# jcasal-homer/HomerHEVC

Hardware: AMD Instinct MI355X
Metric: encoded frames/sec, 1080p & 2160p YUV420 fixed-QP IPPP, 1/2/4/8 MI355X (higher is better)
Workload: dtype int16; 1 GPU; cfg2-1080p-encode; sequences_per_gpu=256, width=1920, height=1080, wfpp_num_threads=17, qp=32, gop=IPPP intra_period=100

## Files before the change

### homerhevc_amd/csrc/enc/enc_common.h

```cpp
#pragma once
#include "enc_prims.h"
#if !defined(__HIPCC__)
#include <stdio.h>
#include <stdlib.h>
#endif

#if !defined(__HIPCC__) && defined(HENC_TRACE_ENABLE)
#include <stdio.h>
extern "C" FILE *henc_trace_file;
#define HENC_TRACE(...) do { if (henc_trace_file) fprintf(henc_trace_file, __VA_ARGS__); } while (0)
#define HENC_TRACE_PW(e, tag)                                                                                                                      \
	do {                                                                                                                                       \
		if (henc_trace_file) {                                                                                                             \
			unsigned a_[3] = {0, 0, 0};                                                                                                \
			for (int c_ = 0; c_ < 3; c_++) {                                                                                           \
				const int n_ = c_ ? 32 : 64;                                                                                       \
				const pred_t *p_ = c_ ? (e).w->pred_c[c_ - 1] : (e).w->pred_y;                                                     \
				for (int y_ = 0; y_ < n_; y_++)                                                                                    \
					for (int x_ = 0; x_ < n_; x_++) a_[c_] += (unsigned)(p_[y_ * n_ + x_] & 0xffff) * (unsigned)(1 + ((x_ + 3 * y_) & 7)); \
			}                                                                                                                          \
			fprintf(henc_trace_file, "PW %s ctu=%d pred=%u,%u,%u\n", tag, (e).ctu->ctu_number, a_[0], a_[1], a_[2]);                   \
		}                                                                                                                                  \
	} while (0)
#else
// ... 200 lines not shown
	e.bg_node = -1;
	*mode = uni(b->bg_mode);
	*bits = uni(b->bg_bits);
	return true;
#else
	(void)g; (void)e; (void)ni; (void)mode; (void)bits;
	return false;
#endif
}

#if defined(__HIP_DEVICE_COMPILE__)
#define HENC_HELPERS(e) true
#else
#define HENC_HELPERS(e) false
#endif

template <class G>
HENC_INLINE bool rd_full(const G, const Seq &S) { return G::rdfull && S.rd_mode == RDM_FULL; }

struct DepthState {
	uint32_t bits = 0;
	HENC_INLINE int get(int d) const { return (int)((bits >> (4 * d)) & 15u); }
	HENC_INLINE void set(int d, int v) { bits = (bits & ~(15u << (4 * d))) | ((uint32_t)v << (4 * d)); }
	HENC_INLINE void inc(int d) { bits += 1u << (4 * d); }
};
struct DepthCosts {
	uint32_t v0 = 0, v1 = 0, v2 = 0, v3 = 0, v4 = 0;
	HENC_INLINE uint32_t get(int d) const { return d == 0 ? v0 : (d == 1 ? v1 : (d == 2 ? v2 : (d == 3 ? v3 : v4))); }
	HENC_INLINE void set(int d, uint32_t x) { v0 = d == 0 ? x : v0; v1 = d == 1 ? x : v1; v2 = d == 2 ? x : v2; v3 = d == 3 ? x : v3; v4 = d == 4 ? x : v4; }
	HENC_INLINE void add(int d, uint32_t x) { set(d, get(d) + x); }
};

struct DepthInts4 {
	int v0 = 0, v1 = 0, v2 = 0, v3 = 0;
	HENC_INLINE int get(int i) const { return i == 0 ? v0 : (i == 1 ? v1 : (i == 2 ? v2 : v3)); }
	HENC_INLINE void set(int i, int x) { v0 = i == 0 ? x : v0; v1 = i == 1 ? x : v1; v2 = i == 2 ? x : v2; v3 = i == 3 ? x : v3; }
	HENC_INLINE void add(int i, int x) { set(i, get(i) + x); }
};

HENC_INLINE int raster2abs(int r)
{
	const int x = r & 15, y = r >> 4;
	int a = 0;
	for (int b = 0; b < 4; b++) a |= (((x >> b) & 1) << (2 * b)) | (((y >> b) & 1) << (2 * b + 1));
	return a;
}
HENC_INLINE int abs2raster(int a)
{
	int x = 0, y = 0;
	for (int b = 0; b < 4; b++) {
		x |= ((a >> (2 * b)) & 1) << b;
		y |= ((a >> (2 * b + 1)) & 1) << b;
	}
	return y * 16 + x;
}
HENC_INLINE Node &node_of(Enc &__restrict__ e, int idx)
{
	HENC_ENC_IN_LDS(e);
#if !defined(__HIPCC__)
	if (idx >= NODES_RESIDENT && node_quadrant(idx) != e.node_quad) {
		fprintf(stderr, "node_of: node %d of quadrant %d while quadrant %d is resident\n", idx, node_quadrant(idx), e.node_quad);
		abort();
	}
#endif
	return e.nodes[node_slot(idx)];
}
HENC_INLINE bool node_is_resident(const Enc &__restrict__ e, int idx) { return idx < NODES_RESIDENT || node_quadrant(idx) == e.node_quad; }
HENC_INLINE void corner_set_left_bottom(Enc &__restrict__ e, int idx, uint8_t v)
{
	HENC_ENC_IN_LDS(e);
	if (node_is_resident(e, idx)) node_of(e, idx).left_bottom_nb = v;
	else e.ctu_g->nodes[idx].left_bottom_nb = v;
}
HENC_INLINE void corner_set_top_right(Enc &__restrict__ e, int idx, uint8_t v)
{
	HENC_ENC_IN_LDS(e);
	if (node_is_resident(e, idx)) node_of(e, idx).top_right_nb = v;
	else e.ctu_g->nodes[idx].top_right_nb = v;
}
HENC_INLINE int node_at(const Enc &__restrict__ e, int depth, int position) { return cfg_depth_start(depth) + position; }

HENC_INLINE CtuPublic *ctu_left_of(Enc &__restrict__ e) { return (e.nb_ctus & 1) ? e.ctu_g - 1 : nullptr; }
HENC_INLINE CtuPublic *ctu_top_of(Enc &__restrict__ e) { return (e.nb_ctus & 2) ? e.ctu_g - e.seq->wctu : nullptr; }
HENC_INLINE CtuPublic *ctu_top_right_of(Enc &__restrict__ e) { return (e.nb_ctus & 4) ? e.ctu_g - e.seq->wctu + 1 : nullptr; }
HENC_INLINE CtuPublic *ctu_top_left_of(Enc &__restrict__ e) { return (e.nb_ctus & 8) ? e.ctu_g - e.seq->wctu - 1 : nullptr; }

HENC_INLINE CtuPublic *pu_left(Enc &__restrict__ e, int ni, uint32_t *idx)
{
	HENC_ENC_IN_LDS(e);
	const Geo &gq = e.geo[ni];
	*idx = gq.abs_left;
	return (gq.raster_index & 15) == 0 ? ctu_left_of(e) : e.ctu;
}
HENC_INLINE CtuPublic *pu_left_bottom(Enc &__restrict__ e, int ni, int has_nb, uint32_t *idx)
{
	HENC_ENC_IN_LDS(e);
	const Geo &gq = e.geo[ni];
	if (!has_nb) return nullptr;
	*idx = gq.abs_left_bottom;
	if (gq.raster_index == NPART - 16) return nullptr;
	if ((gq.raster_index & 15) == 0) return ctu_left_of(e);
	if (gq.raster_index >= NPART - 16) return nullptr;
	if (gq.abs_index > gq.abs_left_bottom) return e.ctu;
	return nullptr;
}
HENC_INLINE CtuPublic *pu_top(Enc &__restrict__ e, int ni, uint32_t *idx, int planar_at_ctu_boundary)
{
	HENC_ENC_IN_LDS(e);
	const Geo &gq = e.geo[ni];
	*idx = gq.abs_top;
	if (gq.raster_index < 16) return planar_at_ctu_boundary ? nullptr : ctu_top_of(e);
	return e.ctu;
}
HENC_INLINE CtuPublic *pu_top_right(Enc &__restrict__ e, int ni, int has_nb, uint32_t *idx)
{
	HENC_ENC_IN_LDS(e);
	const Geo &gq = e.geo[ni];
	if (!has_nb) return nullptr;
	*idx = gq.abs_top_right;
	if (gq.raster_index == 15) return ctu_top_right_of(e);
	if (gq.raster_index < 16) return ctu_top_of(e);
	if ((gq.raster_index & 15) == 15) return nullptr;
	if (gq.abs_index > gq.abs_top_right) return e.ctu;
	return nullptr;
}
HENC_INLINE CtuPublic *pu_top_left(Enc &__restrict__ e, int ni, uint32_t *idx)
{
	HENC_ENC_IN_LDS(e);
	const Geo &gq = e.geo[ni];
	*idx = gq.abs_top_left;
	if (gq.raster_index == 0) return ctu_top_left_of(e);
	if (gq.raster_index < 16) return ctu_top_of(e);
	if ((gq.raster_index & 15) == 0) return ctu_left_of(e);
	return e.ctu;
}

template <class G>
HENC_HD void sync_reference_buffs(const G g, Enc &__restrict__ e, int ni, int src_wnd, int dst_wnd)
{
	HENC_ENC_IN_LDS(e);
	PRIM_T0();
	const Geo &q = e.geo[ni];
	const int16_t *s = dec_ptr(*e.w, src_wnd, COMP_Y) + q.y * DEC_STRIDE_Y + q.x;
	int16_t *d = dec_ptr(*e.w, dst_wnd, COMP_Y) + q.y * DEC_STRIDE_Y + q.x;
	const int n = q.size;
	for (int i = g.tid; i < 2 * n - 1; i += g.n) {
		const int off = i < n ? (n - 1) * DEC_STRIDE_Y + i : (i - n) * DEC_STRIDE_Y + n - 1;
		d[off] = s[off];
	}
	g.sync();
	PRIM_END(PP_SYNC);
}
template <class G>
HENC_HD void sync_reference_buffs_range(const G g, Enc &__restrict__ e, int ni, int src_wnd, int first_dst, int last_dst)
{
	HENC_ENC_IN_LDS(e);
	PRIM_T0();
	const Geo &q = e.geo[ni];
	const int16_t *s = dec_ptr(*e.w, src_wnd, COMP_Y) + q.y * DEC_STRIDE_Y + q.x;
	const int n = q.size, base = q.y * DEC_STRIDE_Y + q.x;
	for (int i0 = g.tid; i0 < 2 * n - 1; i0 += 2 * g.n) {
		const int i1 = i0 + g.n;
		const int off0 = i0 < n ? (n - 1) * DEC_STRIDE_Y + i0 : (i0 - n) * DEC_STRIDE_Y + n - 1;
		const int off1 = i1 < n ? (n - 1) * DEC_STRIDE_Y + i1 : (i1 - n) * DEC_STRIDE_Y + n - 1;
		const bool two = i1 < 2 * n - 1;
		const int16_t v0 = s[off0], v1 = two ? s[off1] : (int16_t)0;
		for (int wnd = first_dst; wnd <= last_dst; wnd++) {
			int16_t *d = dec_ptr(*e.w, wnd, COMP_Y) + base;
			d[off0] = v0;
			if (two) d[off1] = v1;
		}
	}
	g.sync();
	PRIM_END(PP_SYNC);
}
template <class G>
HENC_HD void sync_reference_buffs_chroma(const G g, Enc &__restrict__ e, int ni, int src_wnd, int dst_wnd)
{
	HENC_ENC_IN_LDS(e);
	PRIM_T0();
	const Geo &q = e.geo[ni];
	const int n = q.size_chroma;
	const int16_t *su = dec_ptr(*e.w, src_wnd, COMP_U) + q.yc * DEC_STRIDE_C + q.xc, *sv = dec_ptr(*e.w, src_wnd, COMP_V) + q.yc * DEC_STRIDE_C + q.xc;
	int16_t *du = dec_ptr(*e.w, dst_wnd, COMP_U) + q.yc * DEC_STRIDE_C + q.xc, *dv = dec_ptr(*e.w, dst_wnd, COMP_V) + q.yc * DEC_STRIDE_C + q.xc;
	for (int i = g.tid; i < 2 * n - 1; i += g.n) {
		const int off = i < n ? (n - 1) * DEC_STRIDE_C + i : (i - n) * DEC_STRIDE_C + n - 1;
		const int16_t a = su[off], b = sv[off];
		du[off] = a;
		dv[off] = b;
	}
	g.sync();
	PRIM_END(PP_SYNC);
}
template <class G>
HENC_HD void sync_cu_comp(const G g, Enc &__restrict__ e, int ni, int q_src, int q_dst, int d_src, int d_dst, int comp)
{
	HENC_ENC_IN_LDS(e);
	PRIM_T0();
	const Geo &q = e.geo[ni];
	const int n = comp == COMP_Y ? q.size : q.size_chroma, x = comp == COMP_Y ? q.x : q.xc, y = comp == COMP_Y ? q.y : q.yc;
	const int st = dec_stride(comp), off = comp == COMP_Y ? (q.abs_index << 4) : ((q.abs_index << 4) >> 2);
	const int16_t *ds = dec_ptr(*e.w, d_src, comp) + y * st + x;
	int16_t *dd = dec_ptr(*e.w, d_dst, comp) + y * st + x;
	const int16_t *qs = tq_ptr(*e.w, q_src, comp) + off;
	int16_t *qd = tq_ptr(*e.w, q_dst, comp) + off;
	const int ln = ilog2i(n);
	constexpr int BATCH = 4;
	for (int i0 = g.tid * 4; i0 < n * n; i0 += g.n * 4 * BATCH) {
		S4 a[BATCH], b[BATCH];
#pragma unroll
		for (int u = 0; u < BATCH; u++) {
			const int i = i0 + u * g.n * 4;
			if (i < n * n) {
				a[u] = ld4(ds + (i >> ln) * st + (i & (n - 1)));
				b[u] = ld4(qs + i);
			}
		}
#pragma unroll
		for (int u = 0; u < BATCH; u++) {
			const int i = i0 + u * g.n * 4;
			if (i < n * n) {
				st4(dd + (i >> ln) * st + (i & (n - 1)), a[u]);
				st4(qd + i, b[u]);
			}
		}
	}
	g.sync();
	PRIM_END(PP_SYNC);
}
template <class G>
HENC_HD void sync_cu_chroma_both(const G g, Enc &__restrict__ e, int ni, int q_src, int q_dst, int d_src, int d_dst)
{
	HENC_ENC_IN_LDS(e);
	PRIM_T0();
	const Geo &q = e.geo[ni];
	const int n = q.size_chroma, st = DEC_STRIDE_C, off = (q.abs_index << 4) >> 2, ln = ilog2i(n);
	const int16_t *ds[2], *qs[2];
	int16_t *dd[2], *qd[2];
	for (int c = 0; c < 2; c++) {
		ds[c] = dec_ptr(*e.w, d_src, COMP_U + c) + q.yc * st + q.xc;
		dd[c] = dec_ptr(*e.w, d_dst, COMP_U + c) + q.yc * st + q.xc;
		qs[c] = tq_ptr(*e.w, q_src, COMP_U + c) + off;
		qd[c] = tq_ptr(*e.w, q_dst, COMP_U + c) + off;
	}
	constexpr int BATCH = 2;
	for (int i0 = g.tid * 4; i0 < n * n; i0 += g.n * 4 * BATCH) {
		S4 a[2][BATCH], b[2][BATCH];
#pragma unroll
		for (int u = 0; u < BATCH; u++) {
			const int i = i0 + u * g.n * 4;
			if (i < n * n)
				for (int c = 0; c < 2; c++) {
					a[c][u] = ld4(ds[c] + (i >> ln) * st + (i & (n - 1)));
					b[c][u] = ld4(qs[c] + i);
				}
		}
#pragma unroll
		for (int u = 0; u < BATCH; u++) {
			const int i = i0 + u * g.n * 4;
			if (i < n * n)
				for (int c = 0; c < 2; c++) {
					st4(dd[c] + (i >> ln) * st + (i & (n - 1)), a[c][u]);
					st4(qd[c] + i, b[c][u]);
				}
		}
	}
	g.sync();
	PRIM_END(PP_SYNC);
}
template <class G>
HENC_HD void sync_motion_buffers_luma(const G g, Enc &__restrict__ e, int ni, int q_src, int q_dst, int d_src, int d_dst)
{
	HENC_ENC_IN_LDS(e);
	sync_cu_comp(g, e, ni, q_src, q_dst, d_src, d_dst, COMP_Y);
}
template <class G>
HENC_HD void sync_motion_buffers_chroma(const G g, Enc &__restrict__ e, int ni, int q_src, int q_dst, int d_src, int d_dst)
{
	HENC_ENC_IN_LDS(e);
	sync_cu_comp(g, e, ni, q_src, q_dst, d_src, d_dst, COMP_U);
	sync_cu_comp(g, e, ni, q_src, q_dst, d_src, d_dst, COMP_V);
}

template <class G>
HENC_HD void sync_motion_buffers(const G g, Enc &__restrict__ e, int ni, int q_src, int q_dst, int d_src, int d_dst)
{
	HENC_ENC_IN_LDS(e);
	if (HENC_HELPERS(e)) {
		if (NHELP >= 2) {
			helper_post(g, e, 0, HJOB_SYNC_CU, ni, COMP_U, q_src, q_dst, d_src, d_dst);
			helper_post(g, e, NHELP - 1, HJOB_SYNC_CU, ni, COMP_V, q_src, q_dst, d_src, d_dst);
		} else helper_post(g, e, 0, HJOB_SYNC_CU, ni, COMP_UV, q_src, q_dst, d_src, d_dst);
		sync_cu_comp(g, e, ni, q_src, q_dst, d_src, d_dst, COMP_Y);
		for (int h = 0; h < NHELP; h++) helper_wait(g, e, h);
		return;
	}
	sync_motion_buffers_luma(g, e, ni, q_src, q_dst, d_src, d_dst);
	sync_motion_buffers_chroma(g, e, ni, q_src, q_dst, d_src, d_dst);
}

template <class G>
HENC_HD void nodes_quad_move(const G g, Enc &__restrict__ e, int quad, int to_record)
{
	HENC_ENC_IN_LDS(e);
	constexpr int W3 = (int)(sizeof(Node) * NODE_QUAD_D3 / 4), W4 = (int)(sizeof(Node) * NODE_QUAD_D4 / 4);
	uint32_t *f3 = (uint32_t *)&e.nodes[NODES_RESIDENT], *f4 = (uint32_t *)&e.nodes[NODES_RESIDENT + NODE_QUAD_D3];
	uint32_t *r3 = (uint32_t *)(e.ctu_g->nodes + NODES_RESIDENT + NODE_QUAD_D3 * quad), *r4 = (uint32_t *)(e.ctu_g->nodes + NODES_D3 + NODE_QUAD_D4 * quad);
	for (int i = g.tid; i < W3 + W4; i += g.n) {
		if (to_record) { if (i < W3) r3[i] = f3[i]; else r4[i - W3] = f4[i - W3]; }
		else { if (i < W3) f3[i] = r3[i]; else f4[i - W3] = r4[i - W3]; }
	}
	g.sync();
}
template <class G>
HENC_HD void nodes_select_quad(const G g, Enc &__restrict__ e, int quad)
{	quad = uni(quad);

	HENC_ENC_IN_LDS(e);
	if (quad == e.node_quad) return;
	g.sync();
	if (e.node_quad >= 0) nodes_quad_move(g, e, e.node_quad, 1);
	nodes_quad_move(g, e, quad, 0);
	e.node_quad = quad;
}
template <class G>
HENC_HD void nodes_write_back(const G g, Enc &__restrict__ e)
{
	HENC_ENC_IN_LDS(e);
	g.sync();
	lin_copy_words(g, (const uint32_t *)&e.nodes[0], (uint32_t *)e.ctu_g->nodes, (int)(sizeof(Node) * NODES_RESIDENT / 4));
	if (e.node_quad >= 0) nodes_quad_move(g, e, e.node_quad, 1);
}

HENC_INLINE double calc_mv_correction(uint32_t qp, double avg_dist) { return qp * hclip(avg_dist / 2000., .15, 1.4); }
HENC_INLINE double depth_term(double avg_dist, int depth) { return (hclip(avg_dist - 400, 40., avg_dist) / 1.75) * depth; }
HENC_INLINE double cost_rd(double avg_dist, uint32_t sum) { return hclip(avg_dist / 1.75, 0., 20000.) * sum; }

}
```

### homerhevc_amd/csrc/enc/enc_ctu.h

```cpp
#pragma once
#include "enc_intra.h"
#include "enc_inter.h"
#include "enc_quad.h"

namespace henc {

template <class G>
HENC_HD void info_buffs_copy(const G g, Enc &__restrict__ e, int depth, int abs_idx, int num, int to_ctu)
{
	HENC_ENC_IN_LDS(e);
	PRIM_T0();
	Work &w = *e.w;
	CtuPublic &c = *e.ctu;
	for (int i = g.tid; i < num; i += g.n) {
		const int k = abs_idx + i;
		if (to_ctu) {
			c.cbf[0][k] = w.cbf_buffs[0][depth][k];
			c.cbf[1][k] = w.cbf_buffs[1][depth][k];
			c.cbf[2][k] = w.cbf_buffs[2][depth][k];
			c.tr_idx[k] = w.tr_idx_buffs[depth][k];
			c.intra_mode[0][k] = w.intra_mode_buffs[0][depth][k];
			c.intra_mode[1][k] = w.intra_mode_buffs[1][depth][k];
		} else {
			const uint8_t v0 = c.cbf[0][k], v1 = c.cbf[1][k], v2 = c.cbf[2][k], v3 = c.tr_idx[k], v4 = c.intra_mode[0][k], v5 = c.intra_mode[1][k];
			w.cbf_buffs[0][depth][k] = v0;
			w.cbf_buffs[1][depth][k] = v1;
			w.cbf_buffs[2][depth][k] = v2;
			w.tr_idx_buffs[depth][k] = v3;
			w.intra_mode_buffs[0][depth][k] = v4;
			w.intra_mode_buffs[1][depth][k] = v5;
		}
	}
	g.sync();
	PRIM_END(PP_INFO);
}

template <class G>
HENC_HD void set_inter_info_buffs(const G g, Enc &__restrict__ e, int ni)
{
	HENC_ENC_IN_LDS(e);
	PRIM_T0();
	const Geo &q = e.geo[ni];
	const Node &nd = node_of(e, ni);
	CtuPublic &c = *e.ctu;
	const int a = q.abs_index, n = q.num_part;
	if (nd.prediction_mode == PM_INTER) {
		for (int i = g.tid; i < n; i += g.n) {
			c.inter_mode[a + i] = (uint8_t)nd.inter_mode;
			c.skipped[a + i] = (uint8_t)nd.skipped;
			c.merge[a + i] = (uint8_t)nd.merge_flag;
			c.merge_idx[a + i] = (uint8_t)nd.merge_idx;
			c.mv_ref_idx[a + i] = (int8_t)nd.inter_ref_index;
			if (nd.inter_mode & 1) c.mv_ref[a + i] = nd.inter_mv;
		}
		if (nd.inter_mode & 1) {
			c.mv_diff_ref_idx[a] = (uint8_t)nd.best_candidate_idx;
			c.mv_diff[a] = nd.best_dif_mv;
		}
	} else {
		for (int i = g.tid; i < n; i += g.n) {
			c.mv_ref_idx[a + i] = -1;
			c.skipped[a + i] = 0;
			c.merge[a + i] = 0;
		}
	}
	for (int i = g.tid; i < n; i += g.n) c.pred_mode[a + i] = (uint8_t)nd.prediction_mode;
	g.sync();
	PRIM_END(PP_INFO);
}

template <class G>
HENC_HD void get_back_consolidated_info(const G g, Enc &__restrict__ e, int ni, int depth)
{	ni = uni(ni); depth = uni(depth);

	HENC_ENC_IN_LDS(e);
	info_buffs_copy(g, e, depth, e.geo[ni].abs_index, e.geo[ni].num_part, 0);
	sync_motion_buffers(g, e, ni, 0, depth + 1, 0, depth + 1);
}
template <class G>
HENC_HD void put_consolidated_info(const G g, Enc &__restrict__ e, int ni, int depth)
{	ni = uni(ni); depth = uni(depth);

	HENC_ENC_IN_LDS(e);
	info_buffs_copy(g, e, depth, e.geo[ni].abs_index, e.geo[ni].num_part, 1);
	sync_motion_buffers(g, e, ni, depth + 1, 0, depth + 1, 0);
}

template <class G>
HENC_HD bool consolidate_prediction_info(const G g, Enc &__restrict__ e, int pi, uint32_t parent_cost, uint32_t children_cost, int is_max_depth)
{	pi = uni(pi); parent_cost = uni(parent_cost); children_cost = uni(children_cost); is_max_depth = uni(is_max_depth);

	HENC_ENC_IN_LDS(e);
	const Geo &pq = e.geo[pi];
	Node &pn = node_of(e, pi);
	CtuPublic &c = *e.ctu;
	const int abs_index = pq.abs_index, num = pq.num_part, curr_depth = pq.depth + 1;
	uint32_t children_sum = 0;
	if (pq.child[0] >= 0)
		children_sum = node_of(e, pq.child[0]).sum + node_of(e, pq.child[1]).sum + node_of(e, pq.child[2]).sum + node_of(e, pq.child[3]).sum;
	if (children_cost < parent_cost || !(pn.b_inside && pn.r_inside)) {
		const int part2 = curr_depth < CFG_MAX_PRED_DEPTH ? PART_2Nx2N : PART_NxN;
		pn.cost = children_cost;
		pn.distortion = node_of(e, pq.child[0]).distortion + node_of(e, pq.child[1]).distortion + node_of(e, pq.child[2]).distortion + node_of(e, pq.child[3]).distortion;
		pn.sum = children_sum;
		if (is_max_depth) {
			sync_motion_buffers(g, e, pi, curr_depth + 1, 0, curr_depth + 1, 0);
			info_buffs_copy(g, e, curr_depth, abs_index, num, 1);
			for (int k = 0; k < 4; k++) {
				const int ci = pq.child[k];
				set_inter_info_buffs(g, e, ci);
				const Geo &cq = e.geo[ci];
				const uint8_t qp = (uint8_t)node_of(e, ci).qp;
				for (int i = g.tid; i < cq.num_part; i += g.n) c.qp[cq.abs_index + i] = qp;
			}
			for (int i = g.tid; i < num; i += g.n) {
				c.pred_depth[abs_index + i] = (uint8_t)(curr_depth - (part2 == PART_NxN));
				c.part_size_type[abs_index + i] = (uint8_t)part2;
			}
			g.sync();
		}
		return true;
	} else {
		const int part2 = pq.depth < CFG_MAX_PRED_DEPTH ? PART_2Nx2N : PART_NxN;
		const int parent_depth = pq.depth;
		sync_motion_buffers(g, e, pi, parent_depth + 1, 0, parent_depth + 1, 0);
		info_buffs_copy(g, e, parent_depth, abs_index, num, 1);
		set_inter_info_buffs(g, e, pi);
		const uint8_t qp = (uint8_t)pn.qp;
		for (int i = g.tid; i < num; i += g.n) {
			c.qp[abs_index + i] = qp;
			c.pred_depth[abs_index + i] = (uint8_t)(pq.depth - (part2 == PART_NxN));
			c.part_size_type[abs_index + i] = (uint8_t)part2;
		}
		g.sync();
	}
	return false;
}

template <class G>
HENC_HD void refresh_deeper_windows(const G g, Enc &__restrict__ e, int aux_ni, int from_depth, int with_info)
{	aux_ni = uni(aux_ni); from_depth = uni(from_depth); with_info = uni(with_info);

	HENC_ENC_IN_LDS(e);
	const int max_processing_depth = hmin(CFG_MAX_PRED_DEPTH + e.seq->max_intra_tr_depth - 1, NDEPTH - 1);
	if (from_depth > max_processing_depth) return;
	const Geo &q = e.geo[aux_ni];
	sync_reference_buffs_range(g, e, aux_ni, 0, from_depth + 1, max_processing_depth + 1);
	if (with_info && e.seq->rd_mode != RDM_DIST_ONLY)
		for (int aux_depth = from_depth; aux_depth <= max_processing_depth; aux_depth++) info_buffs_copy(g, e, aux_depth, q.abs_index, q.num_part, 0);
	sync_reference_buffs_chroma(g, e, aux_ni, 0, NWND - 1);
}

template <class G>
HENC_WALK_FN HENC_HD uint32_t encode_intra(const G g, Enc &__restrict__ e, int curr_depth, int position, int part_size_type)
{
	HENC_ENC_IN_LDS(e);
	uint32_t cost = 0;
	if (part_size_type == PART_2Nx2N) {
		uint32_t cl, cc;
		{ HENC_PROF_T0(); cl = encode_intra_luma(g, e, curr_depth, position, part_size_type); HENC_PROF_ADD(e, PF_INTRA_TU); } HENC_TRACE_PW(e, "iluma");
		{ HENC_PROF_T0(); cc = encode_intra_chroma(g, e, curr_depth, position, part_size_type); HENC_PROF_ADD(e, PF_INTRA_CHROMA); } HENC_TRACE_PW(e, "ichroma");
		cost = cl + cc;
	} else {
		for (int n = 0; n < 4; n++) {
			node_of(e, node_at(e, curr_depth, position) + n).qp = (uint32_t)e.ctu_qp;
			cost += encode_intra_luma(g, e, curr_depth, position + n, part_size_type); HENC_TRACE_PW(e, "iluma");
		}
		cost += encode_intra_chroma(g, e, curr_depth, position, part_size_type); HENC_TRACE_PW(e, "ichroma");
	}
	return cost;
}

template <class G>
HENC_WALK_FN HENC_HD uint32_t check_rd_cost_merge(const G g, Enc &__restrict__ e, int depth, int position)
{
	HENC_ENC_IN_LDS(e);
	Work &w = *e.w;
	const Seq &S = *e.seq;
	const int ni = node_at(e, depth, position);
	const Geo &q = e.geo[ni];
	Node &nd = node_of(e, ni);
	CtuPublic &c = *e.ctu;
	const int abs_index = q.abs_index, curr_depth = q.depth, n = q.size, nc = q.size_chroma;
	const int gx = e.ctu_x + q.x, gy = e.ctu_y + q.y;
	int merge_cand_buffer[5] = {0, 0, 0, 0, 0};
	int best_is_skip = 0, best_candidate = 0, have_ctu_cbf = 0, prev_nores_ran = 0;
	uint32_t dist, best_dist = MAX_COST, cost, best_cost = MAX_COST, best_sum = 0, ctu_cbf = 0;
	MV best_mv = {0, 0};
	int best_ref_idx = 0;
	uint8_t inter_modes[5] = {255, 255, 255, 255, 255};
	const double weight = e.f->chroma_weight;
	HENC_QPROF_T0();
	{ PRIM_T0(); get_merge_candidates(e, ni, w.merge_cands, inter_modes); PRIM_END(PP_CAND); }
	if (q.size == 8) HENC_QPROF_MARK(e, 1);
#if defined(HENC_QUAD)
	{
		const QuadCands mc = quad_load_cands(e);
		const int slots = q.size == 8 ? quad_prepare<8>(g, e, ni, mc HENC_QPROF_PASS) : (q.size == 16 ? quad_prepare<16>(g, e, ni, mc HENC_QPROF_PASS) : -1);
		if (slots >= 0) {
			const uint32_t best = q.size == 8 ? quad_merge_loop<8>(g, e, ni, slots, mc, inter_modes HENC_QPROF_PASS) : quad_merge_loop<16>(g, e, ni, slots, mc, inter_modes HENC_QPROF_PASS);
			HENC_QPROF_MARK(e, 7);
			if (g.tid == 0 && e.prof) e.prof[8] += 1;
			return best;
		}
	}
#endif
	for (int cand = 0; cand < CFG_NUM_MERGE_CAND; cand++) {
		int mc_done = 0;
		if (cand >= 1 && w.merge_cands.mv[cand].x == w.merge_cands.mv[cand - 1].x && w.merge_cands.mv[cand].y == w.merge_cands.mv[cand - 1].y &&
		    w.merge_cands.ref_idx[cand] == w.merge_cands.ref_idx[cand - 1]) {
			const int coded_runs = !best_is_skip;
			if (coded_runs) merge_cand_buffer[cand] = merge_cand_buffer[cand - 1];
			const int nores_runs = !(coded_runs && merge_cand_buffer[cand] == 1);
			if (!nores_runs || prev_nores_ran) {
				if (nores_runs) {
					nd.inter_cbf[0] = nd.inter_cbf[1] = nd.inter_cbf[2] = 0;
					nd.inter_tr_idx = 0;
					nd.sum = 0;
				}
				prev_nores_ran = nores_runs;
				continue;
			}
		}
		int coded_ran = 0;
		prev_nores_ran = 0;
		for (int no_res = 0; no_res < 2; no_res++) {
			if (no_res == 1 && merge_cand_buffer[cand] == 1) continue;
			if (best_is_skip && no_res == 0) continue;
			if (no_res == 1) prev_nores_ran = 1;
			if (!mc_done) {
				const MV mv = w.merge_cands.mv[cand];
				const int xlow = -S.margin_y, xhigh = S.width + S.margin_y, ylow = -S.margin_y, yhigh = S.height + S.margin_y;
				const int spx = gx + mv.x / 4, spy = gy + mv.y / 4;
				if (!(spx < xlow || spx + n > xhigh || spy < ylow || spy + n > yhigh)) motion_compensate_cu(g, e, ni, mv);
				else e.n_stale_pred++;
				mc_done = 1;
			}
			if (no_res == 0) {
				cost = dist = encode_inter(g, e, curr_depth, position, PART_2Nx2N); HENC_TRACE_PW(e, "einter");
				cost = (uint32_t)((double)cost + cost_rd(e.f->avg_dist, nd.sum));
				coded_ran = e.inter_ssq_valid;
			} else if (coded_ran) {
				dist = e.inter_ssq[0];
				dist += (uint32_t)(weight * e.inter_ssq[1]);
				dist += (uint32_t)(weight * e.inter_ssq[2]);
				nd.inter_cbf[0] = nd.inter_cbf[1] = nd.inter_cbf[2] = 0;
				nd.inter_tr_idx = 0;
				nd.sum = 0;
				cost = dist;
			} else {
				if (HENC_HELPERS(e)) {
					if (NHELP >= 2) {
						helper_post(g, e, 0, HJOB_SSD, ni, COMP_U);
						helper_post(g, e, NHELP - 1, HJOB_SSD, ni, COMP_V);
					} else helper_post(g, e, 0, HJOB_SSD, ni, COMP_UV);
				}
				dist = blk_ssd(g, w.curr_y + q.y * 64 + q.x, 64, w.pred_y + q.y * 64 + q.x, 64, n);
				if (HENC_HELPERS(e)) {
					for (int h = 0; h < NHELP; h++) helper_wait(g, e, h);
					dist += (uint32_t)(weight * e.box->r[0][0]);
					dist += (uint32_t)(weight * (NHELP >= 2 ? e.box->r[NHELP - 1][0] : e.box->r[0][1]));
				} else {
					dist += (uint32_t)(weight * blk_ssd(g, w.curr_c[0] + q.yc * 32 + q.xc, 32, w.pred_c[0] + q.yc * 32 + q.xc, 32, nc));
					dist += (uint32_t)(weight * blk_ssd(g, w.curr_c[1] + q.yc * 32 + q.xc, 32, w.pred_c[1] + q.yc * 32 + q.xc, 32, nc));
				}
				nd.inter_cbf[0] = nd.inter_cbf[1] = nd.inter_cbf[2] = 0;
				nd.inter_tr_idx = 0;
				nd.sum = 0;
				cost = dist;
			}
			if (cost < best_cost) {
				best_mv = w.merge_cands.mv[cand];
				best_ref_idx = w.merge_cands.ref_idx[cand];
				best_candidate = cand;
				best_dist = dist;
				best_cost = cost;
				best_sum = nd.sum;
				if (no_res == 1) {
					blk_copy(g, w.pred_y + q.y * 64 + q.x, 64, dec_ptr(w, curr_depth + 1, COMP_Y) + q.y * DEC_STRIDE_Y + q.x, DEC_STRIDE_Y, n, n);
					for (int k = 0; k < 2; k++)
						blk_copy(g, w.pred_c[k] + q.yc * 32 + q.xc, 32, dec_ptr(w, curr_depth + 1, COMP_U + k) + q.yc * DEC_STRIDE_C + q.xc, DEC_STRIDE_C, nc, nc);
					lin_zero(g, tq_ptr(w, curr_depth + 1, COMP_Y) + (abs_index << 4), n * n);
					lin_zero(g, tq_ptr(w, curr_depth + 1, COMP_U) + ((abs_index << 4) >> 2), nc * nc);
					lin_zero(g, tq_ptr(w, curr_depth + 1, COMP_V) + ((abs_index << 4) >> 2), nc * nc);
					set_enc_info_buffs(g, e, ni, curr_depth);
				}
				put_consolidated_info(g, e, ni, curr_depth);
				ctu_cbf = (uint32_t)w.cbf_buffs[0][curr_depth][abs_index] | w.cbf_buffs[1][curr_depth][abs_index] | w.cbf_buffs[2][curr_depth][abs_index];
				have_ctu_cbf = 1;
				best_is_skip = (ctu_cbf & 1) == 0;
			}
			if (no_res == 0) {
				if (!have_ctu_cbf) { ctu_cbf = (uint32_t)c.cbf[0][abs_index] | c.cbf[1][abs_index] | c.cbf[2][abs_index]; have_ctu_cbf = 1; }
				if (((ctu_cbf >> curr_depth) & 1) == 0) merge_cand_buffer[cand] = 1;
			}
		}
	}
	nd.skipped = best_is_skip;
	nd.inter_mv = best_mv;
	nd.inter_ref_index = best_ref_idx;
	nd.cost = nd.distortion = best_dist;
	nd.merge_flag = 1;
	nd.merge_idx = best_candidate;
	nd.inter_mode = inter_modes[best_candidate];
	nd.sum = best_sum;
	return best_dist;
}

HENC_INLINE double intra_ratio(uint32_t total_intra_partitions, uint32_t total_partitions)
{
	const uint32_t tp = total_partitions == 0 ? 1 : total_partitions;
	return hclip((double)total_intra_partitions / (double)tp, .0, .15);
}
HENC_INLINE double intra_cost_with_ratio(double intra_dist, double ratio, double add, double rd)
{
	double intra_cost = intra_dist * (1.275 - ratio) + add;
	intra_cost += rd;
	return intra_cost;
}

HENC_INLINE int ctu_takes_intra_walk(const FrameCtx &f, int ctu_num)
{
	if (f.slice_type == SLICE_I) return 1;
	if (f.scene_cut_ctu < 0) return 0;
	if (!f.lockstep) return ctu_num > f.scene_cut_ctu;
	return ctu_num != f.scene_cut_ctu && ctu_num % f.wctu + 2 * (ctu_num / f.wctu) >= f.scene_cut_ctu % f.wctu + 2 * (f.scene_cut_ctu / f.wctu);
}
HENC_INLINE int scene_cut_fires(const Seq &S, const FrameCtx &f, uint32_t intra_before, uint32_t parts_before)
{
	return f.scene_cut_allowed && parts_before > (uint32_t)(S.nctu * NPART / 10) && (double)intra_before > (double)parts_before * .7;
}

template <class G>
HENC_HD uint32_t motion_inter_ctu(const G g, Enc &__restrict__ e)
{
	HENC_ENC_IN_LDS(e);
	const Seq &S = *e.seq;
	CtuPublic &c = *e.ctu;
	const double avg_distortion = e.f->avg_dist;
	const int perf_min_depth = S.perf_min_depth, perf_fast_skip = S.perf_fast_skip;
	DepthState depth_state;
	DepthCosts cost_sum;
	int curr_depth = 0, parent = -1, curr = 0;
	double dist = 0, best_cost;
	const int root = 0;
	while (curr_depth != 0 || depth_state.get(curr_depth) != 1) {
		double cost = 0, intra_cost = 0;
		int stop_recursion = 0, is_skipped = 0;
		const Geo &q = e.geo[curr];
		if constexpr (G::bg) bg_quiesce(g, e);
		if (q.depth >= 1) nodes_select_quad(g, e, q.abs_index >> 6);
		Node &nd = node_of(e, curr);
		curr_depth = q.depth;
		const int part_size_type = curr_depth < CFG_MAX_PRED_DEPTH ? PART_2Nx2N : PART_NxN;
		const int num_part_in_cu = q.num_part;
		const int position = q.list_index - cfg_depth_start(curr_depth);
		nd.qp = (uint32_t)e.ctu_qp;
		if (nd.b_inside && nd.r_inside) {
			int mv_cost = 0;
			if (part_size_type == PART_2Nx2N) {
				uint32_t sad = 0, merge_dist = MAX_COST, merge_cost = MAX_COST, merge_sum = 0;
				MV merge_mv = {0, 0};
				int merge_ref_idx = 0, merge_inter_mode = 0;
				const int action = S.me_precision * 2 - 1;
				nd.prediction_mode = PM_INTER;
				if (curr_depth >= perf_min_depth) {
					{ HENC_PROF_T0(); merge_dist = check_rd_cost_merge(g, e, curr_depth, position); HENC_PROF_ADD(e, PF_MERGE); }
					merge_mv = nd.inter_mv;
					merge_ref_idx = nd.inter_ref_index;
					merge_inter_mode = nd.inter_mode;
					merge_sum = nd.sum;
					merge_cost = merge_dist;
					merge_cost += (uint32_t)nd.merge_idx;
					merge_cost = (uint32_t)(merge_cost * 1.1 + depth_term(avg_distortion, curr_depth));
					merge_cost = (uint32_t)((double)merge_cost + cost_rd(e.f->avg_dist, nd.sum));
					cost = merge_cost;
					dist = merge_dist;
					if (nd.skipped) merge_cost = (uint32_t)(merge_cost * .95);
					if (nd.skipped && (double)merge_cost < avg_distortion * NPART / 2.5) is_skipped = 1;
				} else {
					nd.inter_mv.x = nd.inter_mv.y = 0;
					nd.merge_flag = 0;
					nd.skipped = 0;
					cost = nd.cost = merge_cost = MAX_COST;
					dist = nd.distortion = merge_dist = MAX_COST;
					is_skipped = 0;
				}
				if constexpr (G::bg)
					if (NHELP == 1 && perf_fast_skip && curr_depth >= perf_min_depth && !is_skipped && q.size < 32 && !rd_full(g, S) && e.f->lockstep) bg_post(g, e, curr, curr_depth);
				if (curr_depth >= perf_min_depth) {
					if (!is_skipped) sad = (uint32_t)cu_motion_estimation(g, e, curr_depth, position, PART_2Nx2N, action);
					if (!is_skipped && (q.size < 64 || sad < 100u * num_part_in_cu)) {
						{ HENC_PROF_T0(); mv_cost = predict_inter(g, e, curr_depth, position, PART_2Nx2N); HENC_PROF_ADD(e, PF_PRED_INTER); } HENC_TRACE_PW(e, "pred");
						{ HENC_PROF_T0(); dist = (double)(int)encode_inter(g, e, curr_depth, position, PART_2Nx2N); HENC_PROF_ADD(e, PF_ENC_INTER); }
					} else {
						mv_cost = 0;
						dist = MAX_COST;
						nd.sum = 0;
						nd.inter_mv.x = nd.inter_mv.y = 0;
					}
					cost = dist;
					cost += 2 * mv_cost;
					cost = cost * 1.1 + depth_term(avg_distortion, curr_depth);
					cost += cost_rd(e.f->avg_dist, nd.sum);
					if (cost < merge_cost) {
						nd.merge_flag = 0;
						nd.skipped = 0;
					} else {
						nd.inter_mv = merge_mv;
						nd.inter_ref_index = merge_ref_idx;
						nd.inter_mode = merge_inter_mode;
						nd.sum = merge_sum;
						cost = merge_cost;
						dist = merge_dist;
					}
				}
				nd.cost = (uint32_t)cost;
				nd.distortion = (uint32_t)dist;
				HENC_TRACE("CU ctu=%d d=%d abs=%d inter: merge=%d idx=%d skip=%d mv=(%d,%d) cost=%u dist=%u sum=%u\n", c.ctu_number, curr_depth, q.abs_index,
					   nd.merge_flag, nd.merge_idx, nd.skipped, nd.inter_mv.x, nd.inter_mv.y, nd.cost, nd.distortion, nd.sum);
				if (perf_fast_skip && (dist == 0 || (nd.sum < (uint32_t)num_part_in_cu && dist < .25 * avg_distortion * num_part_in_cu) ||
						       (nd.sum == 0 && dist < avg_distortion * num_part_in_cu))) {
					if (nd.merge_flag) get_back_consolidated_info(g, e, curr, curr_depth);
					stop_recursion = 1;
					(void)consolidate_prediction_info(g, e, curr, nd.cost, MAX_COST, 0);
					refresh_deeper_windows(g, e, curr, curr_depth, 1);
				}
				if (perf_fast_skip && (curr_depth >= perf_min_depth && !stop_recursion && !is_skipped && (q.size < 32 || sad > 400u * num_part_in_cu))) {
					const uint32_t inter_sum = nd.sum;
					if (!nd.merge_flag) put_consolidated_info(g, e, curr, curr_depth);
					e.last_slog = -1;
					uint32_t intra_dist;
					{
						uint32_t cl;
						{ HENC_PROF_T0(); cl = encode_intra_luma(g, e, curr_depth, position, PART_2Nx2N); HENC_PROF_ADD(e, PF_INTRA_TU); } HENC_TRACE_PW(e, "iluma");
						const double add_lb = hclip(avg_distortion - 400, 40., avg_distortion) / 1.75 * curr_depth;
						const double lb = intra_cost_with_ratio((double)cl, .15, add_lb, cost_rd(e.f->avg_dist, nd.sum));
						if (!rd_full(g, S) && e.f->lockstep && lb > cost + 1.) intra_dist = cl;
						else {
							uint32_t cc;
							{ HENC_PROF_T0(); cc = encode_intra_chroma(g, e, curr_depth, position, PART_2Nx2N); HENC_PROF_ADD(e, PF_INTRA_CHROMA); } HENC_TRACE_PW(e, "ichroma");
							intra_dist = cl + cc;
						}
					}
#if defined(__HIPCC__) && defined(HENC_PROFILE)
					if (g.tid == 0 && e.timeline && e.timeline[2] == 0) e.timeline[2] = wall_clock64();
#endif
					const double ratio = intra_ratio(e.total_intra_partitions, e.total_partitions);
					const double add = hclip(avg_distortion - 400, 40., avg_distortion) / 1.75 * curr_depth;
					const double rd = cost_rd(e.f->avg_dist, nd.sum);
					intra_cost = intra_cost_with_ratio((double)intra_dist, ratio, add, rd);
					const int take_intra = intra_cost < cost;
					if (e.n_ratio_cmp < MAX_RATIO_CMP) {
						double *lg = e.ctu_g->ratio_cmp + 4 * e.n_ratio_cmp;
						lg[0] = (double)intra_dist; lg[1] = add; lg[2] = rd; lg[3] = cost;
						e.ctu_g->ratio_out[e.n_ratio_cmp] = (uint8_t)take_intra;
						e.ctu_g->ratio_slog[e.n_ratio_cmp] = (int16_t)e.last_slog;
						if (e.last_slog >= 0) e.ctu_g->slog[e.last_slog].has_cmp = 1;
					}
					e.n_ratio_cmp++;
					HENC_TRACE("CU ctu=%d d=%d abs=%d intra: dist=%u cost=%.3f vs %.3f\n", c.ctu_number, curr_depth, q.abs_index, intra_dist, intra_cost, cost);
					if (take_intra) {
						nd.cost = (uint32_t)intra_cost;
						nd.distortion = intra_dist;
						nd.prediction_mode = PM_INTRA;
						nd.merge_flag = 0;
						nd.skipped = 0;
					} else {
						get_back_consolidated_info(g, e, curr, curr_depth);
						nd.cost = (uint32_t)cost;
						nd.distortion = (uint32_t)dist;
						nd.sum = inter_sum;
						nd.prediction_mode = PM_INTER;
					}
				} else if (curr_depth >= perf_min_depth && !stop_recursion) {
					if (nd.merge_flag) get_back_consolidated_info(g, e, curr, curr_depth);
				}
			} else {
				cost = dist = nd.cost = nd.distortion = MAX_COST;
				depth_state.set(curr_depth, 3);
			}
		} else {
			nd.cost = MAX_COST;
		}
		cost_sum.add(curr_depth, nd.cost);
		depth_state.inc(curr_depth);
		if (curr_depth < CFG_MAX_PRED_DEPTH && nd.tl_inside && !stop_recursion) {
			curr_depth++;
			parent = curr;
		} else if (depth_state.get(curr_depth) == 4) {
			while (depth_state.get(curr_depth) == 4 && curr_depth > 0) {
				const int is_max_depth = curr_depth == CFG_MAX_PRED_DEPTH;
				const Geo &pq = e.geo[parent];
				const uint32_t ccost = node_of(e, pq.child[0]).cost + node_of(e, pq.child[1]).cost + node_of(e, pq.child[2]).cost + node_of(e, pq.child[3]).cost;
				cost = ccost;
				depth_state.set(curr_depth, 0);
				best_cost = node_of(e, parent).cost;
				if (consolidate_prediction_info(g, e, parent, (uint32_t)best_cost, (uint32_t)cost, is_max_depth)) cost_sum.add(e.geo[parent].depth, (uint32_t)cost - (uint32_t)best_cost);
				cost_sum.set(curr_depth, 0);
				curr_depth--;
				parent = e.geo[parent].parent;
				if (curr_depth > perf_min_depth && cost_sum.get(curr_depth) > node_of(e, parent).cost && depth_state.get(curr_depth) < 4 && node_of(e, root).b_inside &&
				    node_of(e, root).r_inside)
					depth_state.set(curr_depth, 4);
			}
			const int aux = parent >= 0 ? e.geo[parent].child[(depth_state.get(curr_depth) + 3) & 3] : root;
			refresh_deeper_windows(g, e, aux, curr_depth, 0);
		}
		if (parent >= 0) curr = e.geo[parent].child[depth_state.get(curr_depth)];
	}
	if constexpr (G::bg) bg_quiesce(g, e);
	return node_of(e, root).cost;
}

HENC_INLINE bool rsplit_of(const Work &w, int ni) { return (w.rsplit[ni >> 5] >> (ni & 31)) & 1u; }
template <class G>
HENC_HD void analyse_recursive_info(const G g, Enc &__restrict__ e)
{
	HENC_ENC_IN_LDS(e);
	const Seq &S = *e.seq;
	Work &w = *e.w;
	uint32_t *var = (uint32_t *)(int16_t *)w.pred_aux;
	uint8_t *split = (uint8_t *)(int16_t *)w.delta_u;
	static_assert(NNODES * 4 <= TU_SCRATCH * 2 && NNODES <= TU_SCRATCH * 2, "the analysis works in the TU scratch");
	for (int ni = 0; ni < NNODES; ni++) {
		const Geo &q = e.geo[ni];
		const bool inside = (e.ctu_y + q.y + q.size <= S.height) && (e.ctu_x + q.x + q.size <= S.width);
		uint32_t v = 0;
		if (inside) {
			const int nc = q.size_chroma;
			const uint32_t vy = blk_modified_variance(g, w.curr_y + q.y * CTU_STRIDE_Y + q.x, CTU_STRIDE_Y, q.size, 1) / (uint32_t)(q.size * q.size);
			uint32_t vc = (uint32_t)(1.25 * blk_modified_variance(g, w.curr_c[0] + q.yc * CTU_STRIDE_C + q.xc, CTU_STRIDE_C, nc, 2) / (nc * nc));
			vc += (uint32_t)(1.25 * blk_modified_variance(g, w.curr_c[1] + q.yc * CTU_STRIDE_C + q.xc, CTU_STRIDE_C, nc, 2) / (nc * nc));
			v = vy + vc;
		}
		if (g.tid == 0) { var[ni] = v; split[ni] = inside ? 0 : 1; }
	}
	g.sync();
	for (int depth = CFG_MAX_PRED_DEPTH - 1; depth >= 0; depth--) {
		const int first = cfg_depth_start(depth), count = 1 << (2 * depth);
		for (int k = g.tid; k < count; k += g.n) {
			const int pi = first + k;
			const Geo &pq = e.geo.lane(pi);
			const uint32_t parent_variance = (uint32_t)(.5 + hsqrt((double)var[pi]));
			for (int l = 0; l < 4; l++) {
				const int ci = pq.child[l];
				const uint32_t child_variance = (uint32_t)(.5 + ((double)(depth + 1) / 4.) * hsqrt((double)var[ci]) + 3 * (depth + 1));
				if (parent_variance > child_variance || split[ci]) { split[pi] = 1; break; }
			}
		}
		g.sync();
	}
	for (int base = 0; base < 11 * 32; base += g.n) {
		const int ni = base + g.tid;
		if (G::n >= 64) {
			const uint64_t m = g.ballot(ni < NNODES && split[ni]);
			if (g.tid == 0) { w.rsplit[base >> 5] = (uint32_t)m; if ((base >> 5) + 1 < 11) w.rsplit[(base >> 5) + 1] = (uint32_t)(m >> 32); }
		} else {
			if ((ni & 31) == 0) w.rsplit[ni >> 5] = 0;
			if (ni < NNODES && split[ni]) w.rsplit[ni >> 5] |= 1u << (ni & 31);
		}
	}
	g.sync();
}

template <class G>
HENC_HD uint32_t motion_intra_ctu(const G g, Enc &__restrict__ e)
{
	HENC_ENC_IN_LDS(e);
	const Seq &S = *e.seq;
	CtuPublic &c = *e.ctu;
	DepthState depth_state;
	DepthCosts cost_sum;
	int curr_depth = 0, parent = 0, curr = 0;
	const int initial_depth = 0, initial_position = 0;
	depth_state.set(0, initial_position);
	e.w->thread_seen_intra = 1;
	if (rd_full(g, S)) {
		bytes_set(g, e.wrd->rd_pred_mode, PM_INTRA, NPART);
		e.rd_luma_depth = -1;
		e.rd_chroma_state = 0;
	}
	const bool fastest = S.perf_mode > 2;
	if (fastest) analyse_recursive_info(g, e);
	while (curr_depth != initial_depth || depth_state.get(curr_depth) != initial_position + 1) {
		const Geo &q = e.geo[curr];
		if (q.depth >= 1) nodes_select_quad(g, e, q.abs_index >> 6);
		Node *nd = &node_of(e, curr);
		curr_depth = q.depth;
		const int part_size_type = curr_depth < CFG_MAX_PRED_DEPTH ? PART_2Nx2N : PART_NxN;
		int position = q.list_index - cfg_depth_start(curr_depth);
		double cost_luma = 0, cost_chroma = 0;
		int stop_recursion = 0;
		nd->qp = (uint32_t)e.ctu_qp;
		if (nd->b_inside && nd->r_inside) {
			if (fastest && rsplit_of(*e.w, curr)) {
				nd->cost = MAX_COST;
			} else if (part_size_type == PART_2Nx2N) {
				{ HENC_PROF_T0(); cost_luma = encode_intra_luma(g, e, curr_depth, position, part_size_type); HENC_PROF_ADD(e, PF_INTRA_TU); } HENC_TRACE_PW(e, "iluma");
				{ HENC_PROF_T0(); cost_chroma = encode_intra_chroma(g, e, curr_depth, position, part_size_type); HENC_PROF_ADD(e, PF_INTRA_CHROMA); } HENC_TRACE_PW(e, "ichroma");
				nd->cost = (uint32_t)(cost_luma + cost_chroma);
				cost_sum.add(curr_depth, nd->cost);
				nd->prediction_mode = PM_INTRA;
				HENC_TRACE("ICU ctu=%d d=%d abs=%d cost=%u (l %.0f c %.0f) mode=%d\n", c.ctu_number, curr_depth, q.abs_index, nd->cost, cost_luma, cost_chroma, nd->intra_mode[0]);
			} else {
				cost_luma = 0;
				for (int n = 0; n < 4; n++) {
					Node &sn = node_of(e, curr + n);
					sn.qp = (uint32_t)e.ctu_qp;
					sn.cost = encode_intra_luma(g, e, curr_depth, position + n, part_size_type); HENC_TRACE_PW(e, "iluma");
					cost_luma += sn.cost;
					cost_sum.add(curr_depth, sn.cost);
					sn.prediction_mode = PM_INTRA;
				}
				if (cost_luma < node_of(e, parent).cost && (nd->b_inside && nd->r_inside)) {
					position = e.geo[e.geo[parent].child[0]].list_index - cfg_depth_start(curr_depth);
					cost_chroma = encode_intra_chroma(g, e, curr_depth, position, part_size_type); HENC_TRACE_PW(e, "ichroma");
					nd->cost += (uint32_t)cost_chroma;
					cost_sum.add(curr_depth, (uint32_t)cost_chroma);
				}
				HENC_TRACE("ICU ctu=%d d=%d abs=%d NxN luma=%.0f chroma=%.0f\n", c.ctu_number, curr_depth, q.abs_index, cost_luma, cost_chroma);
				depth_state.set(curr_depth, 3);
			}
		}
		depth_state.inc(curr_depth);
		if (fastest && (!rsplit_of(*e.w, curr) || nd->cost == 0) && part_size_type != PART_NxN && nd->b_inside && nd->r_inside) {
			(void)consolidate_prediction_info(g, e, curr, nd->cost, MAX_COST, 0);
			stop_recursion = 1;
			const int aux = parent >= 0 ? e.geo[parent].child[(depth_state.get(curr_depth) + 3) & 3] : 0;
			refresh_deeper_windows(g, e, aux, curr_depth, 1);
		}
		if (!stop_recursion && curr_depth < CFG_MAX_PRED_DEPTH && nd->tl_inside) {
			curr_depth++;
			parent = curr;
		} else if (depth_state.get(curr_depth) == 4) {
			while (depth_state.get(curr_depth) == 4 && curr_depth > initial_depth) {
				const Geo &pq = e.geo[parent];
				const uint32_t ccost = node_of(e, pq.child[0]).cost + node_of(e, pq.child[1]).cost + node_of(e, pq.child[2]).cost + node_of(e, pq.child[3]).cost;
				const double cost = ccost;
				depth_state.set(curr_depth, 0);
				const double best_cost = node_of(e, parent).cost;
				if (consolidate_prediction_info(g, e, parent, (uint32_t)best_cost, (uint32_t)cost, curr_depth == CFG_MAX_PRED_DEPTH)) cost_sum.add(e.geo[parent].depth, (uint32_t)cost - (uint32_t)best_cost);
				cost_sum.set(curr_depth, 0);
				curr_depth--;
				parent = e.geo[parent].parent;
				if (S.perf_mode <= 2 && curr_depth > 0 && curr_depth < CFG_MAX_PRED_DEPTH && depth_state.get(curr_depth) < 4 && node_of(e, 0).b_inside && node_of(e, 0).r_inside) {
					double totalcost = 0;
					for (int h = 0; h < depth_state.get(curr_depth); h++) totalcost += node_of(e, e.geo[parent].child[h]).cost;
					if (totalcost > node_of(e, parent).cost) depth_state.set(curr_depth, 4);
				}
			}
// ... 212 lines not shown
```

Before: 474.1 frames/s.

## Fuse reference-buffer syncs and skip redundant consolidation copies in CTU search

Merges the luma range sync and the chroma sync into one pass, and fuses the per-depth info buffer copies into a single fan-out loop, so several group barriers are removed. It tracks when a CU was just restored from consolidated state and skips the redundant motion and info copies at parent consolidation. It syncs only luma when the intra path left chroma untouched, and folds the qp/depth/part-size writes into set_inter_info_buffs to save a barrier. The state tracking adds correctness risk: the chroma-untouched and already-consolidated assumptions must hold exactly. The c1 guard depends on the group size G::n.

```diff
diff --git a/homerhevc_amd/csrc/enc/enc_common.h b/homerhevc_amd/csrc/enc/enc_common.h
--- a/homerhevc_amd/csrc/enc/enc_common.h
+++ b/homerhevc_amd/csrc/enc/enc_common.h
@@ -376,42 +376,32 @@
 	PRIM_END(PP_SYNC);
 }
 template <class G>
-HENC_HD void sync_reference_buffs_range(const G g, Enc &__restrict__ e, int ni, int src_wnd, int first_dst, int last_dst)
+HENC_HD void sync_reference_buffs_planes(const G g, Enc &__restrict__ e, int ni, int src_wnd, int first_dst, int last_dst, int chroma_dst)
 {
 	HENC_ENC_IN_LDS(e);
 	PRIM_T0();
 	const Geo &q = e.geo[ni];
-	const int16_t *s = dec_ptr(*e.w, src_wnd, COMP_Y) + q.y * DEC_STRIDE_Y + q.x;
-	const int n = q.size, base = q.y * DEC_STRIDE_Y + q.x;
+	const int n = q.size, base = q.y * DEC_STRIDE_Y + q.x, nc = q.size_chroma, cbase = q.yc * DEC_STRIDE_C + q.xc;
+	const int16_t *s = dec_ptr(*e.w, src_wnd, COMP_Y) + base;
+	const int16_t *su = dec_ptr(*e.w, src_wnd, COMP_U) + cbase, *sv = dec_ptr(*e.w, src_wnd, COMP_V) + cbase;
+	int16_t *du = dec_ptr(*e.w, chroma_dst, COMP_U) + cbase, *dv = dec_ptr(*e.w, chroma_dst, COMP_V) + cbase;
 	for (int i0 = g.tid; i0 < 2 * n - 1; i0 += 2 * g.n) {
 		const int i1 = i0 + g.n;
 		const int off0 = i0 < n ? (n - 1) * DEC_STRIDE_Y + i0 : (i0 - n) * DEC_STRIDE_Y + n - 1;
 		const int off1 = i1 < n ? (n - 1) * DEC_STRIDE_Y + i1 : (i1 - n) * DEC_STRIDE_Y + n - 1;
-		const bool two = i1 < 2 * n - 1;
+		const int offc0 = i0 < nc ? (nc - 1) * DEC_STRIDE_C + i0 : (i0 - nc) * DEC_STRIDE_C + nc - 1;
+		const int offc1 = i1 < nc ? (nc - 1) * DEC_STRIDE_C + i1 : (i1 - nc) * DEC_STRIDE_C + nc - 1;
+		const bool two = i1 < 2 * n - 1, c0 = i0 < 2 * nc - 1, c1 = G::n < 64 && i1 < 2 * nc - 1;
 		const int16_t v0 = s[off0], v1 = two ? s[off1] : (int16_t)0;
+		const int16_t a0 = c0 ? su[offc0] : (int16_t)0, b0 = c0 ? sv[offc0] : (int16_t)0;
+		const int16_t a1 = c1 ? su[offc1] : (int16_t)0, b1 = c1 ? sv[offc1] : (int16_t)0;
 		for (int wnd = first_dst; wnd <= last_dst; wnd++) {
 			int16_t *d = dec_ptr(*e.w, wnd, COMP_Y) + base;
 			d[off0] = v0;
 			if (two) d[off1] = v1;
 		}
-	}
-	g.sync();
-	PRIM_END(PP_SYNC);
-}
-template <class G>
-HENC_HD void sync_reference_buffs_chroma(const G g, Enc &__restrict__ e, int ni, int src_wnd, int dst_wnd)
-{
-	HENC_ENC_IN_LDS(e);
-	PRIM_T0();
-	const Geo &q = e.geo[ni];
-	const int n = q.size_chroma;
-	const int16_t *su = dec_ptr(*e.w, src_wnd, COMP_U) + q.yc * DEC_STRIDE_C + q.xc, *sv = dec_ptr(*e.w, src_wnd, COMP_V) + q.yc * DEC_STRIDE_C + q.xc;
-	int16_t *du = dec_ptr(*e.w, dst_wnd, COMP_U) + q.yc * DEC_STRIDE_C + q.xc, *dv = dec_ptr(*e.w, dst_wnd, COMP_V) + q.yc * DEC_STRIDE_C + q.xc;
-	for (int i = g.tid; i < 2 * n - 1; i += g.n) {
-		const int off = i < n ? (n - 1) * DEC_STRIDE_C + i : (i - n) * DEC_STRIDE_C + n - 1;
-		const int16_t a = su[off], b = sv[off];
-		du[off] = a;
-		dv[off] = b;
+		if (c0) { du[offc0] = a0; dv[offc0] = b0; }
+		if (c1) { du[offc1] = a1; dv[offc1] = b1; }
 	}
 	g.sync();
 	PRIM_END(PP_SYNC);
diff --git a/homerhevc_amd/csrc/enc/enc_ctu.h b/homerhevc_amd/csrc/enc/enc_ctu.h
--- a/homerhevc_amd/csrc/enc/enc_ctu.h
+++ b/homerhevc_amd/csrc/enc/enc_ctu.h
@@ -36,7 +36,30 @@
 }
 
 template <class G>
-HENC_HD void set_inter_info_buffs(const G g, Enc &__restrict__ e, int ni)
+HENC_HD void info_buffs_fan_out(const G g, Enc &__restrict__ e, int first_depth, int last_depth, int abs_idx, int num)
+{
+	HENC_ENC_IN_LDS(e);
+	PRIM_T0();
+	Work &w = *e.w;
+	CtuPublic &c = *e.ctu;
+	for (int i = g.tid; i < num; i += g.n) {
+		const int k = abs_idx + i;
+		const uint8_t v0 = c.cbf[0][k], v1 = c.cbf[1][k], v2 = c.cbf[2][k], v3 = c.tr_idx[k], v4 = c.intra_mode[0][k], v5 = c.intra_mode[1][k];
+		for (int depth = first_depth; depth <= last_depth; depth++) {
+			w.cbf_buffs[0][depth][k] = v0;
+			w.cbf_buffs[1][depth][k] = v1;
+			w.cbf_buffs[2][depth][k] = v2;
+			w.tr_idx_buffs[depth][k] = v3;
+			w.intra_mode_buffs[0][depth][k] = v4;
+			w.intra_mode_buffs[1][depth][k] = v5;
+		}
+	}
+	g.sync();
+	PRIM_END(PP_INFO);
+}
+
+template <class G>
+HENC_HD void set_inter_info_buffs(const G g, Enc &__restrict__ e, int ni, int pred_depth = -1, int part_size_type = 0)
 {
 	HENC_ENC_IN_LDS(e);
 	PRIM_T0();
@@ -65,17 +88,26 @@
 		}
 	}
 	for (int i = g.tid; i < n; i += g.n) c.pred_mode[a + i] = (uint8_t)nd.prediction_mode;
+	if (pred_depth >= 0) {
+		const uint8_t qp = (uint8_t)nd.qp;
+		for (int i = g.tid; i < n; i += g.n) {
+			c.qp[a + i] = qp;
+			c.pred_depth[a + i] = (uint8_t)pred_depth;
+			c.part_size_type[a + i] = (uint8_t)part_size_type;
+		}
+	}
 	g.sync();
 	PRIM_END(PP_INFO);
 }
 
 template <class G>
-HENC_HD void get_back_consolidated_info(const G g, Enc &__restrict__ e, int ni, int depth)
-{	ni = uni(ni); depth = uni(depth);
+HENC_HD void get_back_consolidated_info(const G g, Enc &__restrict__ e, int ni, int depth, int luma_only = 0)
+{	ni = uni(ni); depth = uni(depth); luma_only = uni(luma_only);
 
 	HENC_ENC_IN_LDS(e);
 	info_buffs_copy(g, e, depth, e.geo[ni].abs_index, e.geo[ni].num_part, 0);
-	sync_motion_buffers(g, e, ni, 0, depth + 1, 0, depth + 1);
+	if (luma_only) sync_motion_buffers_luma(g, e, ni, 0, depth + 1, 0, depth + 1);
+	else sync_motion_buffers(g, e, ni, 0, depth + 1, 0, depth + 1);
 }
 template <class G>
 HENC_HD void put_consolidated_info(const G g, Enc &__restrict__ e, int ni, int depth)
@@ -87,8 +119,8 @@
 }
 
 template <class G>
-HENC_HD bool consolidate_prediction_info(const G g, Enc &__restrict__ e, int pi, uint32_t parent_cost, uint32_t children_cost, int is_max_depth)
-{	pi = uni(pi); parent_cost = uni(parent_cost); children_cost = uni(children_cost); is_max_depth = uni(is_max_depth);
+HENC_HD bool consolidate_prediction_info(const G g, Enc &__restrict__ e, int pi, uint32_t parent_cost, uint32_t children_cost, int is_max_depth, int parent_is_consolidated = 0)
+{	pi = uni(pi); parent_cost = uni(parent_cost); children_cost = uni(children_cost); is_max_depth = uni(is_max_depth); parent_is_consolidated = uni(parent_is_consolidated);
 
 	HENC_ENC_IN_LDS(e);
 	const Geo &pq = e.geo[pi];
@@ -123,16 +155,11 @@
 	} else {
 		const int part2 = pq.depth < CFG_MAX_PRED_DEPTH ? PART_2Nx2N : PART_NxN;
 		const int parent_depth = pq.depth;
-		sync_motion_buffers(g, e, pi, parent_depth + 1, 0, parent_depth + 1, 0);
-		info_buffs_copy(g, e, parent_depth, abs_index, num, 1);
-		set_inter_info_buffs(g, e, pi);
-		const uint8_t qp = (uint8_t)pn.qp;
-		for (int i = g.tid; i < num; i += g.n) {
-			c.qp[abs_index + i] = qp;
-			c.pred_depth[abs_index + i] = (uint8_t)(pq.depth - (part2 == PART_NxN));
-			c.part_size_type[abs_index + i] = (uint8_t)part2;
-		}
-		g.sync();
+		if (!parent_is_consolidated) {
+			sync_motion_buffers(g, e, pi, parent_depth + 1, 0, parent_depth + 1, 0);
+			info_buffs_copy(g, e, parent_depth, abs_index, num, 1);
+		}
+		set_inter_info_buffs(g, e, pi, pq.depth - (part2 == PART_NxN), part2);
 	}
 	return false;
 }
@@ -145,10 +172,8 @@
 	const int max_processing_depth = hmin(CFG_MAX_PRED_DEPTH + e.seq->max_intra_tr_depth - 1, NDEPTH - 1);
 	if (from_depth > max_processing_depth) return;
 	const Geo &q = e.geo[aux_ni];
-	sync_reference_buffs_range(g, e, aux_ni, 0, from_depth + 1, max_processing_depth + 1);
-	if (with_info && e.seq->rd_mode != RDM_DIST_ONLY)
-		for (int aux_depth = from_depth; aux_depth <= max_processing_depth; aux_depth++) info_buffs_copy(g, e, aux_depth, q.abs_index, q.num_part, 0);
-	sync_reference_buffs_chroma(g, e, aux_ni, 0, NWND - 1);
+	sync_reference_buffs_planes(g, e, aux_ni, 0, from_depth + 1, max_processing_depth + 1, NWND - 1);
+	if (with_info && e.seq->rd_mode != RDM_DIST_ONLY) info_buffs_fan_out(g, e, from_depth, max_processing_depth, q.abs_index, q.num_part);
 }
 
 template <class G>
@@ -200,7 +225,9 @@
 		if (slots >= 0) {
 			const uint32_t best = q.size == 8 ? quad_merge_loop<8>(g, e, ni, slots, mc, inter_modes HENC_QPROF_PASS) : quad_merge_loop<16>(g, e, ni, slots, mc, inter_modes HENC_QPROF_PASS);
 			HENC_QPROF_MARK(e, 7);
+#if defined(HENC_QPROF)
 			if (g.tid == 0 && e.prof) e.prof[8] += 1;
+#endif
 			return best;
 		}
 	}
@@ -344,6 +371,7 @@
 	int curr_depth = 0, parent = -1, curr = 0;
 	double dist = 0, best_cost;
 	const int root = 0;
+	int consolidated_cu = -1;
 	while (curr_depth != 0 || depth_state.get(curr_depth) != 1) {
 		double cost = 0, intra_cost = 0;
 		int stop_recursion = 0, is_skipped = 0;
@@ -364,6 +392,7 @@
 				int merge_ref_idx = 0, merge_inter_mode = 0;
 				const int action = S.me_precision * 2 - 1;
 				nd.prediction_mode = PM_INTER;
+				consolidated_cu = -1;
 				if (curr_depth >= perf_min_depth) {
 					{ HENC_PROF_T0(); merge_dist = check_rd_cost_merge(g, e, curr_depth, position); HENC_PROF_ADD(e, PF_MERGE); }
 					merge_mv = nd.inter_mv;
@@ -423,12 +452,14 @@
 						       (nd.sum == 0 && dist < avg_distortion * num_part_in_cu))) {
 					if (nd.merge_flag) get_back_consolidated_info(g, e, curr, curr_depth);
 					stop_recursion = 1;
-					(void)consolidate_prediction_info(g, e, curr, nd.cost, MAX_COST, 0);
+					(void)consolidate_prediction_info(g, e, curr, nd.cost, MAX_COST, 0, nd.merge_flag);
 					refresh_deeper_windows(g, e, curr, curr_depth, 1);
 				}
 				if (perf_fast_skip && (curr_depth >= perf_min_depth && !stop_recursion && !is_skipped && (q.size < 32 || sad > 400u * num_part_in_cu))) {
 					const uint32_t inter_sum = nd.sum;
-					if (!nd.merge_flag) put_consolidated_info(g, e, curr, curr_depth);
+					const int put_here = !nd.merge_flag;
+					int chroma_untouched = 0;
+					if (put_here) put_consolidated_info(g, e, curr, curr_depth);
 					e.last_slog = -1;
 					uint32_t intra_dist;
 					{
@@ -436,7 +467,7 @@
 						{ HENC_PROF_T0(); cl = encode_intra_luma(g, e, curr_depth, position, PART_2Nx2N); HENC_PROF_ADD(e, PF_INTRA_TU); } HENC_TRACE_PW(e, "iluma");
 						const double add_lb = hclip(avg_distortion - 400, 40., avg_distortion) / 1.75 * curr_depth;
 						const double lb = intra_cost_with_ratio((double)cl, .15, add_lb, cost_rd(e.f->avg_dist, nd.sum));
-						if (!rd_full(g, S) && e.f->lockstep && lb > cost + 1.) intra_dist = cl;
+						if (!rd_full(g, S) && e.f->lockstep && lb > cost + 1.) { intra_dist = cl; chroma_untouched = put_here; }
 						else {
 							uint32_t cc;
 							{ HENC_PROF_T0(); cc = encode_intra_chroma(g, e, curr_depth, position, PART_2Nx2N); HENC_PROF_ADD(e, PF_INTRA_CHROMA); } HENC_TRACE_PW(e, "ichroma");
@@ -467,14 +498,15 @@
 						nd.merge_flag = 0;
 						nd.skipped = 0;
 					} else {
-						get_back_consolidated_info(g, e, curr, curr_depth);
+						get_back_consolidated_info(g, e, curr, curr_depth, chroma_untouched);
+						consolidated_cu = curr;
 						nd.cost = (uint32_t)cost;
 						nd.distortion = (uint32_t)dist;
 						nd.sum = inter_sum;
 						nd.prediction_mode = PM_INTER;
 					}
 				} else if (curr_depth >= perf_min_depth && !stop_recursion) {
-					if (nd.merge_flag) get_back_consolidated_info(g, e, curr, curr_depth);
+					if (nd.merge_flag) { get_back_consolidated_info(g, e, curr, curr_depth); consolidated_cu = curr; }
 				}
 			} else {
 				cost = dist = nd.cost = nd.distortion = MAX_COST;
@@ -496,7 +528,8 @@
 				cost = ccost;
 				depth_state.set(curr_depth, 0);
 				best_cost = node_of(e, parent).cost;
-				if (consolidate_prediction_info(g, e, parent, (uint32_t)best_cost, (uint32_t)cost, is_max_depth)) cost_sum.add(e.geo[parent].depth, (uint32_t)cost - (uint32_t)best_cost);
+				if (consolidate_prediction_info(g, e, parent, (uint32_t)best_cost, (uint32_t)cost, is_max_depth, consolidated_cu == parent)) cost_sum.add(e.geo[parent].depth, (uint32_t)cost - (uint32_t)best_cost);
+				consolidated_cu = -1;
 				cost_sum.set(curr_depth, 0);
 				curr_depth--;
 				parent = e.geo[parent].parent;
```

Measured after the change: 491.4 frames/s (median of 6 runs). 3.6% higher.
